# Shinokawa/Fast-SCNN-pytorch

Hardware: AMD Instinct MI355X
Metric: images/sec fwd+bwd @1024x2048 bs=8 per GPU; 1/2/4/8-GPU scaling (higher is better)
Workload: dtype bf16; 1 GPU; cfg3 train step: fwd + CE(ignore -1) + bwd + fused SGD (fused low-res upsample+CE head); model=FastSCNN (19 classes), global_batch=8, per_gpu_batch=8, parallelism=dp1

## Files before the change

### fast-scnn-pytorch_amd/_lib.py

```python
import ctypes
import os
import threading

_HERE = os.path.dirname(os.path.abspath(__file__))
LIB_PATH = os.environ.get("FSCNN_LIB", os.path.join(_HERE, "libfastscnn_hip.so"))

DT_F32, DT_BF16, DT_F16 = 0, 1, 2
DT_U8 = 3

c_int, c_ll, c_float, c_vp, c_char_p = (ctypes.c_int, ctypes.c_longlong, ctypes.c_float,
                                        ctypes.c_void_p, ctypes.c_char_p)
c_ull, c_double = ctypes.c_ulonglong, ctypes.c_double
P_int, P_ll, P_vp = ctypes.POINTER(c_int), ctypes.POINTER(c_ll), ctypes.POINTER(c_vp)
P_float = ctypes.POINTER(c_float)
P_double = ctypes.POINTER(c_double)
c_uint, P_ubyte = ctypes.c_uint, ctypes.POINTER(ctypes.c_ubyte)


class AuxHead(ctypes.Structure):
    _fields_ = [("head", c_int), ("aux_weight", c_float), ("ignore_index", c_ll),
                ("smooth", c_float), ("dice_weight", c_float), ("focal_weight", c_float),
                ("alpha", c_float), ("gamma", c_float), ("thresh", c_float), ("min_kept", c_ll),
                ("class_weight", c_vp)]

# ... 69 lines not shown
                               c_vp]),
    "fscnn_e2e_bev": (c_int, [c_vp, c_int, c_int, c_int, c_int, c_int, c_int, c_int, c_int, c_int,
                              c_int, P_double, c_int, c_int, c_int, c_vp, c_vp, c_vp]),
    "fscnn_forward_e2e_bev": (c_int, [c_vp, c_vp, c_int, c_int, c_int, c_int, c_int, P_float,
                                      P_float, c_int, c_int, c_int, P_double, c_int, c_int, c_int,
                                      c_vp, c_vp, c_vp, c_vp, c_vp, c_vp, c_vp]),
    "fscnn_path_plan": (c_int, [c_vp, c_int, c_int, P_path_params, c_vp, c_vp, c_vp]),
    "fscnn_overlay_mask": (c_int, [c_vp, c_int, c_int, c_int, c_int, c_int, c_vp, c_int, c_int,
                                   P_ubyte, c_vp, c_int, c_float, c_float, c_float, c_vp, c_vp,
                                   c_vp]),
    "fscnn_e2e_overlay": (c_int, [c_vp, c_int, c_int, c_int, c_int, c_int, c_int, c_int, c_int,
                                  c_int, c_int, c_vp, c_int, c_int, c_int, c_int, P_ubyte, c_uint,
                                  c_float, c_float, c_float, c_vp, c_vp, c_vp]),
    "fscnn_forward_e2e_overlay": (c_int, [c_vp, c_vp, c_int, c_int, c_int, c_int, c_int, P_float,
                                          P_float, c_int, c_int, c_int, P_ubyte, c_uint, c_float,
                                          c_float, c_float, c_vp, c_vp, c_vp, c_vp, c_vp, c_vp,
                                          c_vp]),
    "fscnn_seg_metric": (c_int, [c_vp, c_int, c_vp, c_ll, c_int, c_vp, c_vp]),
    "fscnn_forward_aux": (c_int, [c_vp, c_vp, c_int, c_vp, c_vp, c_int, c_vp, c_vp, c_vp, c_vp,
                                  c_ull, c_float, c_float, c_vp]),
    "fscnn_backward_aux": (c_int, [c_vp, c_vp, c_vp, c_vp, c_int, c_vp, c_vp, c_vp, c_vp, c_ull,
                                   c_float, c_int, c_int, c_vp]),
    "fscnn_forward_loss": (c_int, [c_vp, c_vp, c_int, c_vp, c_ll, c_vp, c_vp, c_vp, c_vp, c_vp,
                                   c_ull, c_float, c_float, c_vp]),
    "fscnn_backward_loss": (c_int, [c_vp, c_vp, c_vp, c_vp, c_int, c_vp, c_vp, c_vp, c_vp, c_ull,
                                    c_float, c_int, c_int, c_vp]),
    "fscnn_dice_head_ws_bytes": (c_ll, [c_vp]),
    "fscnn_forward_loss_dice": (c_int, [c_vp, c_vp, c_int, c_vp, c_float, c_float, c_float,
                                        c_float, c_float, c_vp, c_vp, c_vp, c_vp, c_vp, c_vp, c_vp,
                                        c_ull, c_float, c_float, c_vp]),
    "fscnn_backward_loss_dice": (c_int, [c_vp, c_vp, c_vp, c_float, c_float, c_float, c_vp, c_int,
                                         c_vp, c_vp, c_vp, c_vp, c_vp, c_ull, c_float, c_int,
                                         c_int, c_vp]),
    "fscnn_forward_loss_ohem": (c_int, [c_vp, c_vp, c_int, c_vp, c_ll, c_float, c_ll, c_vp, c_vp,
                                        c_vp, c_vp, c_vp, c_vp, c_vp, c_vp, c_vp, c_vp, c_ull,
                                        c_float, c_float, c_vp]),
    "fscnn_aux_head_ws_bytes": (c_ll, [c_vp, c_int]),
    "fscnn_aux_head_ws_offset": (c_ll, [c_vp, c_int, c_char_p, c_int]),
    "fscnn_forward_loss_aux": (c_int, [c_vp, c_vp, c_int, c_vp, P_aux_head, c_vp, c_vp, c_vp, c_vp,
                                       c_vp, c_vp, c_ull, c_float, c_float, c_vp]),
    "fscnn_backward_loss_aux": (c_int, [c_vp, c_vp, P_aux_head, c_vp, c_int, c_vp, c_int, c_vp,
                                        c_vp, c_vp, c_vp, c_vp, c_ull, c_float, c_int, c_int,
                                        c_vp]),
    "fscnn_backward_dx": (c_int, [c_vp, c_vp, c_vp, c_vp, c_vp, c_vp, c_int, c_vp, c_int, c_vp,
                                  c_vp, c_vp, c_vp, c_ull, c_float, c_int, c_int, c_vp]),
    "fscnn_prof_begin": (c_int, [c_int, c_int]),
    "fscnn_prof_end": (c_int, [ctypes.POINTER(ctypes.c_double), P_ll, ctypes.POINTER(ctypes.c_double),
                               ctypes.POINTER(ctypes.c_double)]),
    "fscnn_prof_launch": (c_int, [c_ll, ctypes.POINTER(c_int), ctypes.POINTER(ctypes.c_float),
                                  ctypes.POINTER(ctypes.c_double), ctypes.POINTER(ctypes.c_double),
                                  ctypes.POINTER(c_char_p)]),
    "fscnn_prof_kind_name": (c_char_p, [c_int]),
    "fscnn_ce_parts": (c_ll, [c_int, c_ll]),
    "fscnn_ce_fwd": (c_int, [c_vp, c_int, c_vp, c_int, c_int, c_ll, c_ll, c_vp, c_vp, c_vp]),
    "fscnn_ce_bwd": (c_int, [c_vp, c_int, c_vp, c_int, c_int, c_ll, c_ll, c_vp, c_vp, c_vp,
                             c_vp]),
    "fscnn_sgd": (c_int, [c_vp, c_vp, c_vp, c_ll, c_float, c_float, c_float, c_float, c_int,
                          c_int, c_float, c_vp]),
    "fscnn_adamw": (c_int, [c_vp, c_vp, c_vp, c_vp, c_vp, c_ll, c_double, c_double, c_double,
                            c_double, c_double, c_int, c_int, c_vp, c_int, c_vp, c_vp, c_vp]),
    "fscnn_adamw_segments": (c_int, [c_vp, c_vp, c_vp, c_vp, c_vp, c_vp, c_vp, c_int, c_vp, c_int,
                                     c_vp, c_int, c_vp, c_int, c_int, c_vp, c_vp, c_vp]),
    "fscnn_conv0_fwd": (c_int, [c_vp, c_int, c_int, c_int, c_int, c_vp, c_vp, c_vp, c_int, c_vp,
                                c_int, c_vp]),
    "fscnn_conv0_wgrad_slab_floats": (c_ll, [c_int, c_int, c_int]),
    "fscnn_conv0_wgrad": (c_int, [c_vp, c_int, c_int, c_int, c_int, c_vp, c_int, c_vp, c_vp, c_vp]),
    "fscnn_dw3x3_fwd": (c_int, [c_vp, c_int, c_int, c_int, c_int, c_int, c_int, c_vp, c_vp, c_vp,
                                c_int, c_vp, c_vp]),
    "fscnn_dw3x3_dgrad": (c_int, [c_vp, c_int, c_int, c_int, c_int, c_int, c_int, c_vp, c_vp,
                                  c_vp]),
    "fscnn_dw3x3_wgrad_slab_floats": (c_ll, [c_int, c_int, c_int, c_int, c_int, c_int]),
    "fscnn_dw3x3_wgrad": (c_int, [c_vp, c_vp, c_int, c_int, c_int, c_int, c_int, c_int, c_vp,
                                  c_vp, c_vp]),
    "fscnn_pw_gemm": (c_int, [c_int, c_int, c_int, c_vp, c_int, c_vp, c_int, c_int, c_vp, c_vp,
                              c_vp, c_int, c_int, c_vp, c_int, c_vp, c_int, c_vp]),
    "fscnn_pw_dgrad_bnbwd": (c_int, [c_int, c_int, c_int, c_vp, c_int, c_vp, c_int, c_vp, c_int,
                                     c_vp, c_int, c_vp, c_int, c_vp, c_vp, c_vp, c_vp, c_int,
                                     c_vp, c_vp, c_vp, c_vp, c_vp, c_vp, c_int, P_int, c_vp]),
    "fscnn_kth_smallest": (c_int, [c_vp, c_ll, c_ll, c_vp, c_vp, c_vp]),
    "fscnn_debug_stamps": (c_int, [c_vp, c_int]),
    "fscnn_debug_stamp_count": (c_int, []),
    "fscnn_debug_stamp_tag": (c_char_p, [c_int]),
    "fscnn_pw_wgrad_slab_floats": (c_ll, [c_int, c_int, c_int]),
    "fscnn_pw_gemm_stats_parts": (c_int, [c_int, c_int, c_int, c_int, c_int, c_int]),
    "fscnn_pw_wgrad": (c_int, [c_int, c_int, c_int, c_vp, c_int, c_vp, c_int, c_vp, c_vp, c_int,
                               c_vp]),
    "fscnn_bn_finalize": (c_int, [c_vp, c_int, c_int, c_vp, c_vp, c_vp, c_vp, c_vp, c_float,
                                  c_vp, c_vp, c_vp, c_vp, c_vp]),
    "fscnn_bilinear_ac_fwd": (c_int, [c_vp, c_int, c_int, c_int, c_int, c_int, c_int, c_int,
                                      c_vp, c_int, c_int, c_vp]),
    "fscnn_bilinear_ac_bwd": (c_int, [c_vp, c_int, c_int, c_int, c_int, c_int, c_int, c_int,
                                      c_vp, c_vp, c_vp]),
    "fscnn_pyramid_pool_fwd": (c_int, [c_vp, c_int, c_int, c_int, c_int, c_int, c_int, c_vp,
                                       c_vp]),
    "fscnn_block_ir_fwd": (c_int, [c_vp, c_int, c_int, c_int, c_int, c_int, c_int, c_int, c_int,
                                   c_vp, c_vp, c_vp, c_vp, c_vp, c_vp, c_vp, c_vp, c_vp, c_int,
                                   c_vp, c_int, c_vp]),
    "fscnn_pyramid_pool_bwd": (c_int, [c_vp, c_int, c_int, c_int, c_int, c_int, c_vp, c_int,
                                       c_int, c_vp]),
    "fscnn_bn_apply": (c_int, [c_ll, c_int, c_vp, c_int, c_vp, c_vp, c_vp, c_int, c_vp, c_vp, c_vp,
                               c_int, c_int, c_vp, c_int, c_int, c_vp]),
    "fscnn_bn_bwd": (c_int, [c_ll, c_int, c_vp, c_int, c_vp, c_int, c_vp, c_vp, c_vp, c_vp, c_vp,
                             c_int, c_int, c_vp, c_vp, c_vp, c_vp, c_vp, c_vp, c_vp, c_vp, c_vp,
                             c_vp, c_vp, c_vp, c_vp, c_int, P_int, P_int, c_vp]),
    "fscnn_ppm_branches_ok": (c_int, [c_int, c_int, c_int]),
    "fscnn_ppm_branches_fwd": (c_int, [c_int, P_int, c_int, c_vp, c_vp, c_vp, c_vp, c_vp, c_vp,
                                       c_vp, c_float, c_vp, c_vp, c_int, c_vp, c_vp, c_vp, c_vp,
                                       c_int, c_vp]),
    "fscnn_ppm_branches_bwd": (c_int, [c_int, P_int, c_int, c_vp, c_int, c_vp, c_int, c_vp, c_vp,
                                       c_vp, c_vp, c_vp, c_vp, c_vp, c_vp, c_vp, c_vp, c_vp, c_int,
                                       c_vp]),
    "fscnn_ppm_up_fwd": (c_int, [c_vp, c_int, c_int, c_int, c_int, c_vp, c_int, c_int, c_vp]),
    "fscnn_ppm_up_bwd": (c_int, [c_vp, c_int, c_int, c_int, c_int, c_int, c_int, c_vp, c_vp]),
    "fscnn_dropout": (c_int, [c_vp, c_int, c_int, c_int, c_int, c_int, c_int, c_ull, c_vp, c_ull,
                              c_float, c_vp, c_vp, c_vp, c_int, c_vp]),
    "fscnn_dw3x3_parts": (c_int, [c_int, c_int, c_int, c_int, c_int, c_int, c_int]),
    "fscnn_dw3x3_ct_width": (c_int, [c_int, c_int, c_int, c_int, c_int, c_int]),
    "fscnn_dw3x3_fwd_train": (c_int, [c_vp, c_int, c_int, c_int, c_int, c_int, c_int, c_vp, c_vp,
                                      c_vp, c_vp, c_vp, c_vp, c_vp, c_vp, c_vp, c_vp, c_vp, c_vp,
                                      c_float, c_vp, c_vp, c_vp, c_vp, P_int, c_vp]),
    "fscnn_dw3x3_dgrad_bn": (c_int, [c_vp, c_int, c_int, c_int, c_int, c_int, c_int, c_vp, c_vp,
                                     c_vp, c_vp, c_vp, c_vp, c_vp, c_int, c_vp, c_vp, c_vp, c_vp,
                                     c_vp, c_vp, P_int, c_vp]),
    "fscnn_dw3x3_wgrad_train": (c_int, [c_vp, c_vp, c_int, c_int, c_int, c_int, c_int, c_int,
                                        c_vp, c_vp, c_vp, c_vp, c_vp]),
    "fscnn_pw_fwd_train_route": (c_int, [c_int, c_int, c_int, c_int, c_int, c_int, c_int, P_int]),
    "fscnn_pw_fwd_train": (c_int, [c_int, c_int, c_int, c_vp, c_int, c_vp, c_vp, c_vp, c_int, c_vp,
                                   c_vp, c_int, c_vp, c_vp, c_vp, c_vp, c_vp, c_vp, c_vp, c_vp,
                                   c_float, c_vp, c_vp, c_vp, c_vp, c_int, P_int, P_int, c_vp]),
    "fscnn_pw_wgrad_train": (c_int, [c_int, c_int, c_int, c_vp, c_int, c_vp, c_int, c_vp, c_vp,
                                     c_vp, c_vp, c_vp, c_vp, c_int, P_int, c_vp]),
    "fscnn_pw_dgrad_train_route": (c_int, [c_int, c_int, c_int, c_int, c_int, c_int, c_int, c_int,
                                           P_int]),
    "fscnn_pw_dgrad_train": (c_int, [c_int, c_int, c_int, c_vp, c_int, c_vp, c_int, c_vp, c_int,
                                     c_vp, c_int, c_vp, c_int, c_vp, c_vp, c_vp, c_vp, c_int,
                                     c_vp, c_vp, c_vp, c_vp, c_vp, c_vp, c_vp, c_int, c_float,
                                     c_ull, c_ull, c_vp, c_int, P_int, P_int, c_vp]),
    "fscnn_im2col3": (c_int, [c_vp, c_int, c_int, c_int, c_int, c_int, c_int, c_vp, c_int, c_vp]),
    "fscnn_col2im3": (c_int, [c_vp, c_int, c_int, c_int, c_int, c_int, c_int, c_vp, c_int, c_int,
                              c_vp]),
    "fscnn_block_ir_s2_fwd": (c_int, [c_vp, c_int, c_int, c_int, c_int, c_int, c_int, c_int, c_int,
                                      c_vp, c_vp, c_vp, c_vp, c_vp, c_vp, c_vp, c_vp, c_vp, c_vp,
                                      c_int, c_vp]),
    "fscnn_block_ltd_fwd": (c_int, [c_vp, c_int, c_int, c_int, c_int, c_int, c_vp, c_vp, c_vp,
                                    c_vp, c_vp, c_vp, c_vp, c_vp, c_vp, c_vp, c_int, c_vp]),
    "fscnn_block_dsconv_fwd": (c_int, [c_vp, c_int, c_int, c_int, c_int, c_int, c_int, c_vp, c_vp,
                                       c_vp, c_vp, c_vp, c_vp, c_vp, c_int, c_vp]),
    "fscnn_block_dsconv_res_fwd": (c_int, [c_vp, c_int, c_int, c_int, c_int, c_int, c_int, c_int,
                                           c_int, c_vp, c_vp, c_vp, c_vp, c_vp, c_vp, c_vp, c_int,
                                           c_vp, c_int, c_vp]),
    "fscnn_block_cls_fwd": (c_int, [c_vp, c_int, c_int, c_int, c_int] + [c_vp] * 14 + [c_int, c_vp, c_vp,
                                                                              c_int, c_vp]),
    "fscnn_block_ffm_fwd": (c_int, [c_vp, c_int, c_int, c_int, c_int, c_int, c_int, c_vp, c_int,
                                    c_vp, c_vp, c_vp, c_vp, c_vp, c_vp, c_vp, c_vp, c_vp, c_vp,
                                    c_int, c_vp]),
}

_lib = None
_lock = threading.Lock()


def load():
    global _lib
    if _lib is not None:
        return _lib
    with _lock:
# ... 48 lines not shown
```

### fast-scnn-pytorch_amd/csrc/capi.cpp

```cpp
#include <algorithm>
#include <chrono>
#include <cmath>
#include <cstdlib>
#include <cstdarg>
#include <cstdio>
#include <cstring>
#include <new>
#include <string>

#include "../../include/fastscnn.h"
#include "net.hpp"

namespace fscnn {

static thread_local char g_err[512] = "";

void set_error(const char* fmt, ...) {
  va_list ap;
  va_start(ap, fmt);
  vsnprintf(g_err, sizeof g_err, fmt, ap);
  va_end(ap);
}
const char* last_error() { return g_err; }

// ... 1125 lines not shown
                      int dz_dtype, float* slab, float* dw, void* stream) {
  Conv0WgradArgs a{};
  a.x = x; a.x_bf16 = x_dtype; a.N = N; a.H = H; a.W = W;
  a.Ho = (H - 3) / 2 + 1; a.Wo = (W - 3) / 2 + 1; a.dz = dz; a.slab = slab;
  int rc = conv0_wgrad(a, dz_dtype, S(stream));
  if (rc) return rc;
  return reduce_slabs(slab, conv0_wgrad_parts(N, a.Ho, a.Wo, 0), 864, 864, dw, 0, S(stream));
}

int fscnn_dw3x3_fwd(const void* x, int dtype, int N, int H, int W, int C, int stride,
                    const float* w, const float* scale, const float* shift, int relu, void* y,
                    void* stream) {
  DwArgs a{};
  a.N = N; a.H = H; a.W = W; a.C = C; a.stride = stride;
  a.Ho = (H - 1) / stride + 1; a.Wo = (W - 1) / stride + 1;
  a.x = x; a.w = w; a.scale = scale; a.shift = shift; a.relu = relu; a.y = y;
  return dw_fwd(a, dtype, S(stream));
}
int fscnn_dw3x3_dgrad(const void* dy, int dtype, int N, int H, int W, int C, int stride,
                      const float* w, void* dx, void* stream) {
  DwBwdArgs a{};
  a.N = N; a.H = H; a.W = W; a.C = C; a.stride = stride;
  a.Ho = (H - 1) / stride + 1; a.Wo = (W - 1) / stride + 1;
  a.dy = dy; a.w = w; a.dx = dx;
  return dw_dgrad(a, dtype, S(stream));
}
long long fscnn_dw3x3_wgrad_slab_floats(int N, int H, int W, int C, int stride, int dtype) {
  int Ho = (H - 1) / stride + 1, Wo = (W - 1) / stride + 1;
  return (long long)dw_wgrad_parts(N, Ho, Wo, C, dtype, stride) * 9 * C;
}
int fscnn_dw3x3_wgrad(const void* x, const void* dy, int dtype, int N, int H, int W, int C,
                      int stride, float* slab, float* dw, void* stream) {
  DwBwdArgs a{};
  a.N = N; a.H = H; a.W = W; a.C = C; a.stride = stride;
  a.Ho = (H - 1) / stride + 1; a.Wo = (W - 1) / stride + 1;
  a.x = x; a.dy = dy; a.slab = slab;
  int rc = dw_wgrad(a, dtype, S(stream));
  if (rc) return rc;
  return dw_wgrad_reduce(slab, dw_wgrad_parts(N, a.Ho, a.Wo, C, dtype, stride), C, dw, S(stream));
}

int fscnn_pw_gemm_stats_parts(int M, int N, int K, int lda, int ldc, int dtype) {
  GemmArgs a{};
  static float dummy;
  a.M = M; a.N = N; a.K = K; a.lda = lda; a.ldb = K; a.ldc = ldc; a.part = &dummy;
  return gemm_nt_parts(a, dtype);
}
int fscnn_pw_gemm(int M, int N, int K, const void* A, int lda, const void* B, int ldb,
                  int b_trans, const float* scale, const float* shift, const void* R, int ldr,
                  int relu, void* C, int ldc, float* stats_part, int dtype, void* stream) {
  GemmArgs a{};
  a.M = M; a.N = N; a.K = K; a.A = A; a.lda = lda; a.B = B; a.ldb = ldb; a.b_trans = b_trans;
  a.scale = scale; a.shift = shift; a.R = R; a.ldr = ldr; a.relu = relu; a.C = C; a.ldc = ldc;
  a.part = stats_part;
  return gemm_nt(a, dtype, S(stream));
}
int fscnn_pw_dgrad_bnbwd(int M, int N, int K, const void* D, int ldd, const void* B, int ldb,
                         const void* R, int ldr, void* dX, int lddx, const void* z, int ldz,
                         const float* mean, const float* invstd, const float* scale,
                         const float* shift, int relu_mode, float* part, unsigned* counters,
                         double* tsum, float* dgamma, float* dbeta, float* coef, int dtype,
                         int* path, void* stream) {
  if (!D || !B || !dX || !z || !mean || !invstd || !scale || !shift || !part || !counters ||
      !tsum || !dgamma || !dbeta || !coef) {
    set_error("fscnn_pw_dgrad_bnbwd: null argument");
    return E_INVALID;
  }
  if (dtype < DT_F32 || dtype > DT_F16 || (relu_mode != 0 && relu_mode != 2)) {
    set_error("fscnn_pw_dgrad_bnbwd: dtype %d / relu_mode %d", dtype, relu_mode);
    return E_INVALID;
  }
  GemmArgs a{};
  a.M = M; a.N = N; a.K = K; a.A = D; a.lda = ldd; a.B = B; a.ldb = ldb; a.b_trans = 0;
  a.R = R; a.ldr = ldr; a.C = dX; a.ldc = lddx;
  a.bpart = part; a.bz = z; a.ldbz = ldz;
  a.bmean = mean; a.binvstd = invstd; a.bscale = scale; a.bshift = shift; a.bmode = relu_mode;
  a.tail.counters = counters; a.tail.tsum = tsum; a.tail.count = (double)M;
  a.tail.dgamma = dgamma; a.tail.dbeta = dbeta; a.tail.coef = coef;
  if (path) *path = gemm_stream_ok(a, dtype) ? 1 : 0;
  return gemm_nt(a, dtype, S(stream));
}
long long fscnn_pw_wgrad_slab_floats(int M, int N, int K) {
  return (long long)gemm_tn_splits(M, N, K) * N * K;
}
int fscnn_pw_wgrad(int M, int N, int K, const void* D, int ldd, const void* X, int ldx,
                   float* slab, float* dW, int dtype, void* stream) {
  GemmTnArgs a{};
  a.M = M; a.N = N; a.K = K; a.D = D; a.ldd = ldd; a.X = X; a.ldx = ldx; a.slab = slab;
  int s = gemm_tn_splits(M, N, K);
  int rc = gemm_tn(a, s, dtype, S(stream));
  if (rc) return rc;
  return reduce_slabs(slab, s, (long long)N * K, (long long)N * K, dW, 0, S(stream));
}

int fscnn_bn_finalize(float* part, int P, int C, const float* gamma, const float* beta,
                      float* rmean, float* rvar, long long* nbt, float momentum, float* mean,
                      float* invstd, float* scale, float* shift, void* stream) {
  BnFinalizeArgs a{};
  a.part = part; a.P = P; a.C = C; a.gamma = gamma; a.beta = beta; a.rmean = rmean;
  a.rvar = rvar; a.nbt = nbt; a.momentum = momentum; a.mean = mean; a.invstd = invstd;
  a.scale = scale; a.shift = shift;
  return bn_finalize(a, S(stream));
}

int fscnn_bilinear_ac_fwd(const void* x, int dtype, int N, int Hi, int Wi, int C, int Ho, int Wo,
                          void* y, int out_nchw, int out_dtype, void* stream) {
  UpArgs a{};
  a.N = N; a.Hi = Hi; a.Wi = Wi; a.C = C; a.Ho = Ho; a.Wo = Wo; a.x = x; a.ldx = C; a.y = y;
  a.ldy = C;
  if (out_nchw) return up_nchw(a, dtype, out_dtype, S(stream));
  return up_nhwc(a, dtype, S(stream));
}
int fscnn_bilinear_ac_bwd(const void* dy, int dtype, int N, int Hi, int Wi, int C, int Ho, int Wo,
                          float* tmp, void* dx, void* stream) {
  AxisBwdArgs a{};
  a.n_o1 = (long long)N * Ho; a.n_o2 = 1; a.Lout = Wo; a.Lin = Wi; a.n_in = C;
  a.g = dy; a.g_s1 = (long long)Wo * C; a.g_idx = C; a.g_in = 1;
  a.d = tmp; a.d_s1 = (long long)Wi * C; a.d_idx = C; a.d_in = 1;
  int rc = axis_bwd(a, dtype, DT_F32, S(stream));
  if (rc) return rc;
  AxisBwdArgs b{};
  b.n_o1 = N; b.n_o2 = 1; b.Lout = Ho; b.Lin = Hi; b.n_in = (long long)Wi * C;
  b.g = tmp; b.g_s1 = (long long)Ho * Wi * C; b.g_idx = (long long)Wi * C; b.g_in = 1;
  b.d = dx; b.d_s1 = (long long)Hi * Wi * C; b.d_idx = (long long)Wi * C; b.d_in = 1;
  return axis_bwd(b, DT_F32, dtype, S(stream));
}
int fscnn_pyramid_pool_fwd(const void* x, int dtype, int N, int H, int W, int C, int ldx,
                           void* pooled, void* stream) {
  PoolArgs a{};
  a.N = N; a.H = H; a.W = W; a.C = C; a.x = x; a.ldx = ldx; a.pooled = pooled;
  return pyramid_pool(a, dtype, S(stream));
}
int fscnn_pyramid_pool_bwd(const void* dpooled, int dtype, int N, int H, int W, int C, void* dx,
                           int lddx, int accumulate, void* stream) {
  PoolBwdArgs a{};
  a.N = N; a.H = H; a.W = W; a.C = C; a.dpooled = dpooled; a.dx = dx; a.lddx = lddx;
  a.accumulate = accumulate;
  return pyramid_pool_bwd(a, dtype, S(stream));
}

static bool dt_ok(int dtype) { return dtype >= DT_F32 && dtype <= DT_F16; }
static int vec_w(int dtype) { return dtype == DT_F32 ? 4 : 8; }
static bool ld_ok(int ld, int C, int V) { return ld >= C && ld % V == 0; }

int fscnn_bn_apply(long long M, int C, const void* z, int ldz, const float* scale,
                   const float* shift, const void* z2, int ldz2, const float* scale2,
                   const float* shift2, const void* res, int ldres, int relu, void* y, int ldy,
                   int dtype, void* stream) {
  if (!z || !scale || !shift || !y || (z2 && (!scale2 || !shift2))) {
    set_error("fscnn_bn_apply: null argument");
    return E_INVALID;
  }
  if (!dt_ok(dtype)) {
    set_error("fscnn_bn_apply: dtype %d", dtype);
    return E_INVALID;
  }
  const int V = vec_w(dtype);
  if (M < 1 || C < 1 || C % V || !ld_ok(ldz, C, V) || !ld_ok(ldy, C, V) ||
      (z2 && !ld_ok(ldz2, C, V)) || (res && !ld_ok(ldres, C, V)) ||
      M * (C / V) >= (1LL << 31)) {
    set_error("fscnn_bn_apply: M=%lld C=%d ldz=%d ldz2=%d ldres=%d ldy=%d (C and every row stride "
              "a multiple of %d, strides >= C)", M, C, ldz, ldz2, ldres, ldy, V);
    return E_INVALID;
  }
  BnApplyArgs a{};
  a.M = M; a.C = C;
// ... 826 lines not shown
```

### fast-scnn-pytorch_amd/csrc/gemm.hip

```cpp
#include "bn_finish.hpp"

namespace fscnn {


constexpr int G_BM = 128;
constexpr int G_VROW = 8;
constexpr int G_VPAD = 9;
constexpr int G_ATMAX = 768;

template <typename T>
struct MfmaOp;

template <>
struct MfmaOp<float> {
  static __device__ __forceinline__ void run(const uint4& a, const uint4& b, f32x4& acc) {
    acc = __builtin_amdgcn_mfma_f32_16x16x4f32(__uint_as_float(a.x), __uint_as_float(b.x), acc, 0, 0, 0);
    acc = __builtin_amdgcn_mfma_f32_16x16x4f32(__uint_as_float(a.y), __uint_as_float(b.y), acc, 0, 0, 0);
    acc = __builtin_amdgcn_mfma_f32_16x16x4f32(__uint_as_float(a.z), __uint_as_float(b.z), acc, 0, 0, 0);
    acc = __builtin_amdgcn_mfma_f32_16x16x4f32(__uint_as_float(a.w), __uint_as_float(b.w), acc, 0, 0, 0);
  }
};

template <>
struct MfmaOp<bf16> {
// ... 662 lines not shown
        rx[i][h] = *reinterpret_cast<const uint4*>(X + (okx ? (size_t)m * a.ldx + k : 0));
      }
    }
  };
  float xsc[XT ? V : 1], xsh[XT ? V : 1];
  if constexpr (XT) {
    const int kb = k0 + (tid % VPR) * V;
#pragma unroll
    for (int j = 0; j < V; ++j) {
      const int k = kb + j < a.K ? kb + j : 0;
      xsc[j] = a.x_scale[k];
      xsh[j] = a.x_shift[k];
    }
  }
  auto mask = [&](int mc) {
#pragma unroll
    for (int i = 0; i < PAIRS; ++i) {
      const int id = tid + 256 * i;
      const int rp = id / VPR, vv = id - rp * VPR;
      const int n = n0 + vv * V, k = k0 + vv * V;
#pragma unroll
      for (int h = 0; h < 2; ++h) {
        const bool okm = mc + 2 * rp + h < me;
        uint4 dv = rd[i][h];
        rd[i][h] = zero_tail<T>(dv, okm ? a.N - n : 0);
        uint4 xv = rx[i][h];
        if constexpr (XT) xv = bnrelu_vec<T>(xv, xsc, xsh);
        rx[i][h] = zero_tail<T>(xv, okm ? a.K - k : 0);
      }
    }
  };
  using Pair = typename std::conditional<sizeof(T) == 2, uint32_t, uint2>::type;
  if (mb < me) load(mb);
  for (int mc = mb; mc < me; mc += TN_MC) {
    mask(mc);
    __syncthreads();
#pragma unroll
    for (int i = 0; i < PAIRS; ++i) {
      const int id = tid + 256 * i;
      const int rp = id / VPR, vv = id - rp * VPR;
      const T* d0 = reinterpret_cast<const T*>(&rd[i][0]);
      const T* d1 = reinterpret_cast<const T*>(&rd[i][1]);
      const T* x0 = reinterpret_cast<const T*>(&rx[i][0]);
      const T* x1 = reinterpret_cast<const T*>(&rx[i][1]);
#pragma unroll
      for (int j = 0; j < V; ++j) {
        const int n = vv * V + j;
        const int off = n * LD + swz(n, 2 * rp);
        Pair pd, px;
        __builtin_memcpy(reinterpret_cast<T*>(&pd), d0 + j, sizeof(T));
        __builtin_memcpy(reinterpret_cast<T*>(&pd) + 1, d1 + j, sizeof(T));
        __builtin_memcpy(reinterpret_cast<T*>(&px), x0 + j, sizeof(T));
        __builtin_memcpy(reinterpret_cast<T*>(&px) + 1, x1 + j, sizeof(T));
        *reinterpret_cast<Pair*>(&sDt[off]) = pd;
        *reinterpret_cast<Pair*>(&sXt[off]) = px;
      }
    }
    __syncthreads();
    if (mc + TN_MC < me) load(mc + TN_MC);
#pragma unroll
    for (int ks = 0; ks < TN_MC / 32; ++ks) {
      const int kb = ks * 32 + 8 * lq;
#pragma unroll
      for (int i = 0; i < 2; ++i)
#pragma unroll
        for (int j = 0; j < 2; ++j) {
          const int na = wn + i * 16 + li, nb = wk + j * 16 + li;
          TnOps<T>::mma(&sDt[na * LD + swz(na, kb)], &sXt[nb * LD + swz(nb, kb)], acc[i][j]);
        }
    }
  }
  float* sl = a.slab + (size_t)split * a.N * a.K;
#pragma unroll
  for (int i = 0; i < 2; ++i)
#pragma unroll
    for (int j = 0; j < 2; ++j)
#pragma unroll
      for (int r = 0; r < 4; ++r) {
        int n = n0 + wn + i * 16 + lq * 4 + r, k = k0 + wk + j * 16 + li;
        if (n < a.N && k < a.K) sl[(size_t)n * a.K + k] = acc[i][j][r];
      }
}

int gemm_tn_splits(int M, int N, int K) {
  constexpr int target = 512;
  int tiles = cdiv(N, TN_T) * cdiv(K, TN_T);
  int s = target / tiles;
  int smax = cdiv(M, 4 * TN_MC);
  if (s > smax) s = smax;
  if (s >= 8) s &= ~7;
  if (s < 1) s = 1;
  return s;
}

int gemm_tn(GemmTnArgs a, int splits, int dtype, hipStream_t st) {
  const int V = dtype == DT_F32 ? 4 : 8;
  if (a.ldd % V || a.ldx % V || (uintptr_t)a.D % 16 || (uintptr_t)a.X % 16) {
    set_error("gemm_tn: operands must be 16-B aligned (ldd=%d ldx=%d)", a.ldd, a.ldx);
    return E_INVALID;
  }
  a.rows_per_split = cdiv(cdiv(a.M, splits), TN_MC) * TN_MC;
  a.splits = splits;
  dim3 grid(cdiv(a.N, TN_T) * cdiv(a.K, TN_T) * splits);
  const double E = dtype == DT_F32 ? 4.0 : 2.0;
  const double M = a.M, N = a.N, K = a.K;
  ProfScope ps(PK_GEMM_TN, st, E * (M * N + M * K) + 4.0 * N * K, 2.0 * M * N * K);
  const bool xt = a.x_scale != nullptr;
  if (xt && (!a.x_shift || a.K % V)) {
    set_error("gemm_tn: lazy BN on X needs x_shift and K %% %d == 0", V);
    return E_UNSUPPORTED;
  }
#define TN_LAUNCH(T)                                        \
  do {                                                      \
    if (xt) prof_launch(gemm_tn_kernel<T, true>, grid, 256, 0, st, a); \
    else prof_launch(gemm_tn_kernel<T, false>, grid, 256, 0, st, a);   \
  } while (0)
  if (dtype == DT_F32) TN_LAUNCH(float);
  else if (dtype == DT_F16) TN_LAUNCH(f16);
  else TN_LAUNCH(bf16);
#undef TN_LAUNCH
  return check_launch("gemm_tn");
}

constexpr int RED_Q = 64;

__global__ void reduce_fold_kernel(float* slab, int S, int Q, long long stride, int count) {
  int i = blockIdx.x * blockDim.x + threadIdx.x;
  int q = blockIdx.y;
  if (i >= count) return;
  float s = 0.f;
  for (int k0 = q; k0 < S; k0 += 8 * Q) {
    float v[8];
#pragma unroll
    for (int u = 0; u < 8; ++u) {
      const int k = k0 + u * Q;
      const float t = slab[(size_t)(k < S ? k : q) * stride + i];
      v[u] = k < S ? t : 0.f;
    }
#pragma unroll
    for (int u = 0; u < 8; ++u) s += v[u];
  }
  slab[(size_t)q * stride + i] = s;
}

__global__ void reduce_final_kernel(const float* slab, int S, long long stride, int count,
                                    float* out, int accumulate, int C9) {
  int i = blockIdx.x * blockDim.x + threadIdx.x;
  if (i >= count) return;
  float s = 0.f;
  for (int k0 = 0; k0 < S; k0 += 8) {
    float v[8];
#pragma unroll
    for (int u = 0; u < 8; ++u) {
      const float t = slab[(size_t)(k0 + u < S ? k0 + u : 0) * stride + i];
      v[u] = k0 + u < S ? t : 0.f;
    }
#pragma unroll
    for (int u = 0; u < 8; ++u) s += v[u];
  }
  int o = C9 ? (i % C9) * 9 + i / C9 : i;
  out[o] = accumulate ? out[o] + s : s;
}

int reduce_slabs_ex(float* slab, int S, long long stride, long long count, float* out,
                    int accumulate, int C9, hipStream_t st) {
  if (count <= 0 || count > 0x7fffffff) { set_error("reduce_slabs: bad count"); return E_INVALID; }
  int n = (int)count;
  int S2 = S;
  if (S > RED_Q) {
    dim3 g1(cdiv(n, 256), RED_Q);
    prof_launch(reduce_fold_kernel, g1, 256, 0, st, slab, S, RED_Q, stride, n);
    S2 = RED_Q;
  }
  prof_launch(reduce_final_kernel, cdiv(n, 256), 256, 0, st, slab, S2, stride, n, out, accumulate, C9);
  return check_launch("reduce_slabs");
}

int reduce_slabs(float* slab, int S, long long stride, long long count, float* out,
                 int accumulate, hipStream_t st) {
  return reduce_slabs_ex(slab, S, stride, count, out, accumulate, 0, st);
}

__device__ __forceinline__ int red_job(const RedTable& t, int b) {
  int lo = 0, hi = t.n - 1;
  while (lo < hi) {
    const int mid = (lo + hi + 1) >> 1;
    if (t.blk0[mid] <= b) lo = mid;
    else hi = mid - 1;
  }
  return lo;
}

__global__ void reduce_fold_multi_kernel(RedTable t) {
  const int jb = red_job(t, blockIdx.x);
  const RedJob& J = t.j[jb];
  const int nb = cdiv(J.count, 256);
  const int local = blockIdx.x - t.blk0[jb];
  const int q = local / nb;
  const int i = (local - q * nb) * blockDim.x + threadIdx.x;
  if (i >= J.count) return;
  float s = 0.f;
  for (int k0 = q; k0 < J.S; k0 += 8 * J.Q) {
// ... 95 lines not shown
```

### fast-scnn-pytorch_amd/csrc/kernels.hpp

```cpp
#pragma once
#include "common.hpp"

struct fscnn_path_params;

namespace fscnn {

constexpr int MAX_FOLD = 48;
constexpr double BN_FROZEN_COUNT = -1.0;


struct Conv0Args {
  const void* x;
  int x_bf16;
  int N, H, W, Ho, Wo;
  const float* w;
  const float* scale;
  const float* shift;
  int relu;
  void* y;
  float* part;
  unsigned long long* stamps = nullptr;
};

struct Conv0WgradArgs {
// ... 436 lines not shown
  const float *scp, *shp;
  void* y; int ldy;
  const void* r = nullptr;
  int ldr = 0;
  int rs;
  const void* wc = nullptr;
  const float* bc = nullptr;
  int ncls = 0;
  void* logits = nullptr; int ldl = 0;
  int Hi = 0, Wi = 0;
  const void* xh = nullptr;
  int ldxh = 0;
  const void* wh = nullptr;
  const float *sch = nullptr, *shh = nullptr;
  unsigned long long* stamps = nullptr;
};
bool ds_ok(const DsArgs& a);
struct Ds2Args {
  const void* x;
  int N, H, W, Ho, Wo;
  const float* wd;
  const float *scd, *shd;
  const void* wp;
  const float *scp, *shp;
  void* y; int ldy;
  unsigned long long* stamps = nullptr;
};
bool ds2_ok(const Ds2Args& a);
int ds2_fwd(const Ds2Args& a, int dtype, hipStream_t st);
int ds_rows(int N, int H, int W);
int ds_fwd(const DsArgs& a, int dtype, hipStream_t st);

struct Conv0DgradArgs {
  const void* dz;
  const float* w;
  int N, H, W, Ho, Wo;
  void* dx;
  int dx_dtype;
};
int conv0_dgrad(const Conv0DgradArgs& a, int dz_dtype, hipStream_t st);
int conv0_parts(int N, int Ho, int Wo);
int conv0_fwd(const Conv0Args& a, int y_dtype, hipStream_t st);
int conv0_wgrad_parts(int N, int Ho, int Wo, int rows_per_block);
int conv0_wgrad(const Conv0WgradArgs& a, int dz_dtype, hipStream_t st);

constexpr int LC0_SLAB = 2 * 864 + 27;
struct LtdC0BwdArgs {
  int N, H, W;
  int Ho, Wo;
  const void* dy;
  const float* w;
  BnBwdPart bs{};
  BnTail tail{};
  const void* x;
  int x_dtype, XH, XW;
  float* slab;
};
int ltd_c0_bwd_parts(int N, int H, int W);
bool ltd_c0_bwd_ok(int dtype, int x_dtype, int XW, const void* x);
int ltd_c0_bwd(const LtdC0BwdArgs& a, int dtype, hipStream_t st);
int conv0_wgrad_combine(const float* sums, const float* tab, const float* mean, float* dw,
                        hipStream_t st);

int dw_parts(int N, int Ho, int Wo, int C, int dtype, int stride);
int dw_ct_width(int N, int Ho, int Wo, int W, int C, int dtype, int stride);
int dw_fwd(const DwArgs& a, int dtype, hipStream_t st);
int dw_dgrad(const DwBwdArgs& a, int dtype, hipStream_t st);
int dw_dgrad_parts(int N, int H, int W, int C, int dtype, int stride);
int dw_fwd_tail_ink(const DwArgs& a, int dtype, int* P);
int dw_dgrad_tail_ink(const DwBwdArgs& a, int dtype, int* P);
int dw_wgrad_parts(int N, int Ho, int Wo, int C, int dtype, int stride);
int dw_wgrad(const DwBwdArgs& a, int dtype, hipStream_t st);
int dw_wgrad_reduce(float* slab, int P, int C, float* dw, hipStream_t st);

int gemm_parts(int M);
int gemm_nt(const GemmArgs& a, int dtype, hipStream_t st);
bool gemm_stream_ok(const GemmArgs& a, int dtype);
int gemm_stream(const GemmArgs& a, int dtype, hipStream_t st);
int gemm_stream_parts(const GemmArgs& a, int dtype);
int gemm_nt_parts(const GemmArgs& a, int dtype);
int gemm_nt_tail_ink(const GemmArgs& a, int dtype, int* P);
int gemm_tn_splits(int M, int N, int K);
int gemm_tn(GemmTnArgs a, int splits, int dtype, hipStream_t st);
int reduce_slabs(float* slab, int S, long long stride, long long count, float* out,
                 int accumulate, hipStream_t st);
int reduce_slabs_ex(float* slab, int S, long long stride, long long count, float* out,
                    int accumulate, int C9, hipStream_t st);
constexpr int RED_MAXJOBS = 64;
struct RedJob {
  float* slab;
  float* out;
  long long stride;
  int S, count, accumulate, C9;
  int Q = 0;
};
struct RedTable {
  int n = 0;
  int blocks = 0;
  int blk0[RED_MAXJOBS + 1] = {};
  RedJob j[RED_MAXJOBS];
};
int reduce_slabs_multi(const RedTable& t, hipStream_t st);
int colsum_parts(int M);
int colsum(const void* D, int M, int N, int ld, float* part, int dtype, hipStream_t st);

int bn_fold(const FoldTable& t, hipStream_t st);
int bn_finalize(const BnFinalizeArgs& a, hipStream_t st);
int bn_apply(const BnApplyArgs& a, int dtype, hipStream_t st);
int bn_bwd_parts(long long M, int C, int dtype, int* rows_per_block);
int bn_bwd_reduce(const BnBwdArgs& a, int dtype, hipStream_t st);
int bn_bwd_finalize(float* part, int P, int C, double count, float* dgamma, float* dbeta,
                    float* coef, hipStream_t st, unsigned* counters = nullptr,
                    const BnBwdTab& tab = BnBwdTab());
int bn_bwd_apply(const BnBwdArgs& a, int dtype, hipStream_t st);

int up_nhwc(const UpArgs& a, int dtype, hipStream_t st);
int up_nchw(const UpArgs& a, int in_dtype, int out_dtype, hipStream_t st);
bool up_nchw_rows_path(const UpArgs& a);
int up_argmax(const UpArgs& a, int in_dtype, void* labels, int label_u8, hipStream_t st);
int seg_metric(const void* pred, int pred_u8, const long long* target, long long n, int C,
               long long* counts, hipStream_t st);
int axis_bwd(const AxisBwdArgs& a, int g_dtype, int d_dtype, hipStream_t st);
int pyramid_pool(const PoolArgs& a, int dtype, hipStream_t st);
int pyramid_pool_bwd(const PoolBwdArgs& a, int dtype, hipStream_t st);
int ppm_up_fwd(const PpmUpArgs& a, int dtype, hipStream_t st);
int ppm_up_bwd(const PpmUpArgs& a, void* dfeats, int dtype, hipStream_t st);

bool ppm_branches_ok(int maxM, int K, int dtype);
int ppm_branches_fwd(const PpmFwdArgs& a, int dtype, hipStream_t st);
int ppm_branches_bwd(const PpmBwdArgs& a, int dtype, hipStream_t st);

int ce_parts(int N, long long HW);
int ce_fwd(const CeArgs& a, float* out, int dtype, hipStream_t st);
int ce_bwd(const CeArgs& a, const float* gout, const float* stats, int dtype, hipStream_t st);
int ohem_prob(const CeArgs& a, float thresh, float* prob, unsigned long long* counts, int dtype,
              hipStream_t st);
int ohem_threshold_dev(const float* key, long long n, const unsigned long long* counts,
                       long long min_kept, float thresh, unsigned* work, float* thr,
                       hipStream_t st);
int dice_loss_fwd(const void* logits, int dtype, const long long* target, int N, int C, long long HW,
                  float alpha, float gamma, int focal, float* part, double* stats, hipStream_t st);
int dice_loss_bwd(const void* logits, int dtype, const long long* target, int N, int C, long long HW,
                  float alpha, float gamma, int focal, const double* stats, const float* gout,
                  float smooth, float wd, float wf, void* dlogits, hipStream_t st);
int ce_head_parts(int N, int Hl, int Wl);
int ce_head(const CeHeadArgs& a, float* out2, int dtype, hipStream_t st);
bool ce_head2_form(int C, int ldl, int dtype);
bool ce_head_reads_tgt8(int C, int ldl, int W, int dtype);
int ce_pack_targets(const long long* t, long long n, int C, long long ignore_index,
                    signed char* out, hipStream_t st);
int ce_head_scale(const float* g_raw, void* g, long long M, int C, int ld, const float* gout,
                  const float* out2, int dtype, hipStream_t st, float weight = 1.f);
int aux_loss_combine(const float* main, const float* aux, float aux_weight, float* out3,
                     hipStream_t st);
long long dice_head_ws_bytes(int N, int Hl, int Wl, int C, int ldl);
int dice_head(const DiceHeadArgs& a, void* head_ws, float* loss, double* stats, int dtype,
              hipStream_t st);
int dice_head_scale(const void* head_ws, void* g, long long M, int C, int ld, const float* gout,
                    const double* stats, float smooth, float wd, float wf, double npix, int dtype,
                    hipStream_t st, float weight = 1.f);
bool ohem_head_ok(int C);
int ohem_head(const OhemHeadArgs& a, long long min_kept, unsigned* work, float* out2, int dtype,
              hipStream_t st);
int eval_head_parts(int N, int H, int W);
bool eval_head_ok(int N, int C, int Hl, int Wl, int H, int W, int dice);
int eval_head(const EvalHeadArgs& a, int dtype, hipStream_t st);
// ... 92 lines not shown
```

### include/fastscnn.h

```cpp
#ifndef FASTSCNN_H
#define FASTSCNN_H

#ifdef __cplusplus
extern "C" {
#endif

typedef struct fscnn_net fscnn_net;
typedef struct fscnn_plan fscnn_plan;

const char* fscnn_version(void);
const char* fscnn_last_error(void);

int fscnn_net_create(int num_classes, int aux, fscnn_net** out);
void fscnn_net_destroy(fscnn_net* net);
int fscnn_net_param_count(const fscnn_net* net, int* count, long long* total_floats);
int fscnn_net_param_info(const fscnn_net* net, int i, const char** name, long long* offset,
                         long long* numel);
int fscnn_net_buffer_count(const fscnn_net* net, int* count, long long* total_floats, int* num_bn);
int fscnn_net_buffer_info(const fscnn_net* net, int i, const char** name, long long* offset,
                          long long* numel);
int fscnn_net_stage_range(const fscnn_net* net, int stage, long long* begin, long long* end);

int fscnn_plan_create(const fscnn_net* net, int N, int H, int W, int dtype, int train,
                      fscnn_plan** out);
// ... 237 lines not shown
                               const void* res, int ldres, void* y, int ldy, void* stream);

int fscnn_block_cls_fwd(const void* x, int dtype, int N, int H, int W, const float* w_dw1,
                        const float* scale_d1, const float* shift_d1, const void* w_pw1,
                        const float* scale_p1, const float* shift_p1, const float* w_dw2,
                        const float* scale_d2, const float* shift_d2, const void* w_pw2,
                        const float* scale_p2, const float* shift_p2, const void* w_cls,
                        const float* b_cls, int ncls, void* tmp, void* logits, int ldl,
                        void* stream);

int fscnn_block_ffm_fwd(const void* low, int dtype, int N, int Hi, int Wi, int H, int W,
                        const void* high, int ldhigh, const float* w_dw, const float* scale_d,
                        const float* shift_d, const void* w_low, const float* scale_l,
                        const float* shift_l, const void* w_high, const float* scale_h,
                        const float* shift_h, void* y, int ldy, void* stream);

int fscnn_prof_begin(int kind, int max_launches);
int fscnn_prof_end(double* total_ms, long long* launches, double* bytes, double* flops);
int fscnn_prof_launch(long long i, int* kind, float* ms, double* bytes, double* flops,
                      const char** layer);
const char* fscnn_prof_kind_name(int kind);
int fscnn_debug_stamps(void* buf, int max_launches);
int fscnn_debug_stamp_count(void);
const char* fscnn_debug_stamp_tag(int i);

long long fscnn_ce_parts(int N, long long HW);
int fscnn_ce_fwd(const void* logits, int dtype, const long long* target, int N, int C,
                 long long HW, long long ignore_index, float* part, float* out2, void* stream);
int fscnn_ce_bwd(const void* logits, int dtype, const long long* target, int N, int C,
                 long long HW, long long ignore_index, const float* grad_out,
                 const float* out2, void* dlogits, void* stream);
int fscnn_sgd(float* p, const float* g, float* buf, long long n, float lr, float momentum,
              float dampening, float weight_decay, int nesterov, int first, float grad_scale,
              void* stream);

int fscnn_adamw(float* p, const float* g, float* exp_avg, float* exp_avg_sq,
                float* max_exp_avg_sq, long long n, double lr, double beta1, double beta2,
                double eps, double weight_decay, int amsgrad, int maximize, float* step, int tick,
                const float* grad_scale, const float* found_inf, void* stream);
#define FSCNN_ADAMW_CHUNK 2048
#define FSCNN_ADAMW_MAX_GROUPS 8
typedef struct fscnn_adamw_seg {
  long long begin, end;
  int group;
  int chunk0;
} fscnn_adamw_seg;
typedef struct fscnn_adamw_group {
  double lr, beta1, beta2, eps, weight_decay;
  int amsgrad, maximize;
  int step_slot;
} fscnn_adamw_group;
int fscnn_adamw_segments(float* p, const float* g, float* exp_avg, float* exp_avg_sq,
                         float* max_exp_avg_sq, const fscnn_adamw_seg* segs,
                         const fscnn_adamw_seg* host_segs, int nseg, const int* chunk_seg,
                         int nchunks, const fscnn_adamw_group* groups, int ngroups, float* steps,
                         int nslots, int tick, const float* grad_scale, const float* found_inf,
                         void* stream);

int fscnn_conv0_fwd(const void* x, int x_dtype, int N, int H, int W, const float* w,
                    const float* scale, const float* shift, int relu, void* y, int y_dtype,
                    void* stream);
long long fscnn_conv0_wgrad_slab_floats(int N, int H, int W);
int fscnn_conv0_wgrad(const void* x, int x_dtype, int N, int H, int W, const void* dz,
                      int dz_dtype, float* slab, float* dw, void* stream);
int fscnn_dw3x3_fwd(const void* x, int dtype, int N, int H, int W, int C, int stride,
                    const float* w, const float* scale, const float* shift, int relu, void* y,
                    void* stream);
int fscnn_dw3x3_dgrad(const void* dy, int dtype, int N, int H, int W, int C, int stride,
                      const float* w, void* dx, void* stream);
long long fscnn_dw3x3_wgrad_slab_floats(int N, int H, int W, int C, int stride, int dtype);
int fscnn_dw3x3_wgrad(const void* x, const void* dy, int dtype, int N, int H, int W, int C,
                      int stride, float* slab, float* dw, void* stream);
int fscnn_pw_gemm_stats_parts(int M, int N, int K, int lda, int ldc, int dtype);
int fscnn_pw_gemm(int M, int N, int K, const void* A, int lda, const void* B, int ldb,
                  int b_trans, const float* scale, const float* shift, const void* R, int ldr,
                  int relu, void* C, int ldc, float* stats_part, int dtype, void* stream);
int fscnn_pw_dgrad_bnbwd(int M, int N, int K, const void* D, int ldd, const void* B, int ldb,
                         const void* R, int ldr, void* dX, int lddx, const void* z, int ldz,
                         const float* mean, const float* invstd, const float* scale,
                         const float* shift, int relu_mode, float* part, unsigned* counters,
                         double* tsum, float* dgamma, float* dbeta, float* coef, int dtype,
                         int* path, void* stream);
long long fscnn_pw_wgrad_slab_floats(int M, int N, int K);
int fscnn_pw_wgrad(int M, int N, int K, const void* D, int ldd, const void* X, int ldx,
                   float* slab, float* dW, int dtype, void* stream);
int fscnn_bn_finalize(float* part, int P, int C, const float* gamma, const float* beta,
                      float* rmean, float* rvar, long long* nbt, float momentum, float* mean,
                      float* invstd, float* scale, float* shift, void* stream);
int fscnn_bilinear_ac_fwd(const void* x, int dtype, int N, int Hi, int Wi, int C, int Ho, int Wo,
                          void* y, int out_nchw, int out_dtype, void* stream);
int fscnn_bilinear_ac_bwd(const void* dy, int dtype, int N, int Hi, int Wi, int C, int Ho, int Wo,
                          float* tmp, void* dx, void* stream);
int fscnn_pyramid_pool_fwd(const void* x, int dtype, int N, int H, int W, int C, int ldx,
                           void* pooled, void* stream);
int fscnn_pyramid_pool_bwd(const void* dpooled, int dtype, int N, int H, int W, int C, void* dx,
                           int lddx, int accumulate, void* stream);

int fscnn_bn_apply(long long M, int C, const void* z, int ldz, const float* scale,
                   const float* shift, const void* z2, int ldz2, const float* scale2,
                   const float* shift2, const void* res, int ldres, int relu, void* y, int ldy,
                   int dtype, void* stream);
int fscnn_bn_bwd(long long M, int C, const void* dy, int lddy, const void* mask, int ldmask,
                 const void* z, const float* mean, const float* invstd, const float* scale,
                 const float* shift, int relu_mode, int frozen, const void* z2,
                 const float* mean2, const float* invstd2, const float* scale2, float* part,
                 unsigned* counters, void* dz, void* dz2, float* dgamma, float* dbeta,
                 float* dgamma2, float* dbeta2, float* coef, int dtype, int* P,
                 int* rows_per_block, void* stream);
int fscnn_ppm_branches_ok(int maxM, int K, int dtype);
int fscnn_ppm_branches_fwd(int nb, const int* M, int K, const void* x, const void* w,
                           const float* gamma, const float* beta, float* rmean, float* rvar,
                           long long* nbt, float momentum, void* z, void* y, int ldy, float* mean,
                           float* invstd, float* scale, float* shift, int dtype, void* stream);
int fscnn_ppm_branches_bwd(int nb, const int* M, int K, const void* dy, int lddy, const void* y,
                           int ldy, const void* z, const float* mean, const float* invstd,
                           const float* scale, const float* gamma, const void* x, const void* w,
                           float* dgamma, float* dbeta, float* dw, void* dx, int dtype,
                           void* stream);
int fscnn_ppm_up_fwd(const void* feats, int dtype, int N, int H, int W, void* y, int ldy, int coff,
                     void* stream);
int fscnn_ppm_up_bwd(const void* dy, int dtype, int N, int H, int W, int ldy, int coff,
                     void* dfeats, void* stream);
int fscnn_dropout(const void* x, int ldx, int dtype, int N, int H, int W, int C,
                  unsigned long long seed, const unsigned long long* seed_slot,
                  unsigned long long seed_add, float p, const float* x_scale,
                  const float* x_shift, void* y, int ldy, void* stream);
int fscnn_dw3x3_parts(int N, int H, int W, int C, int stride, int dtype, int dgrad);
int fscnn_dw3x3_ct_width(int N, int H, int W, int C, int stride, int dtype);
int fscnn_dw3x3_fwd_train(const void* x, int dtype, int N, int H, int W, int C, int stride,
                          const float* w, const float* in_scale, const float* in_shift, void* z,
                          float* part, unsigned* counters, double* tsum, const float* gamma,
                          const float* beta, float* rmean, float* rvar, long long* nbt,
                          float momentum, float* mean, float* invstd, float* scale, float* shift,
                          int* in_kernel, void* stream);
int fscnn_dw3x3_dgrad_bn(const void* dy, int dtype, int N, int H, int W, int C, int stride,
                         const float* w, void* dx, const void* z, const float* mean,
                         const float* invstd, const float* scale, const float* shift,
                         int relu_mode, float* part, unsigned* counters, double* tsum,
                         float* dgamma, float* dbeta, float* coef, int* in_kernel, void* stream);
int fscnn_dw3x3_wgrad_train(const void* x, const void* dy, int dtype, int N, int H, int W, int C,
                            int stride, const float* x_scale, const float* x_shift, float* slab,
                            float* dw, void* stream);

int fscnn_pw_fwd_train_route(int M, int N, int K, int lda, int ldc, int lazy, int dtype,
                             int* records);
int fscnn_pw_fwd_train(int M, int N, int K, const void* A, int lda, const float* a_scale,
                       const float* a_shift, const void* B, int ldb, const float* bias, void* z,
                       int ldc, float* part, unsigned* counters, double* tsum, const float* gamma,
                       const float* beta, float* rmean, float* rvar, long long* nbt,
                       float momentum, float* mean, float* invstd, float* scale, float* shift,
                       int dtype, int* route, int* records, void* stream);
int fscnn_pw_wgrad_train(int M, int N, int K, const void* D, int ldd, const void* X, int ldx,
                         const float* x_scale, const float* x_shift, float* slab, float* dW,
                         float* bias_part, float* dbias, int dtype, int* splits, void* stream);
int fscnn_pw_dgrad_train_route(int M, int N, int K, int ldd, int lddx, int residual, int drop_hw,
                               int dtype, int* records);
int fscnn_pw_dgrad_train(int M, int N, int K, const void* D, int ldd, const void* B, int ldb,
                         const void* R, int ldr, void* dX, int lddx, const void* z, int ldz,
                         const float* mean, const float* invstd, const float* scale,
                         const float* shift, int relu_mode, float* part, unsigned* counters,
                         double* tsum, float* dgamma, float* dbeta, float* coef, float* tab,
                         int drop_hw, float drop_p, unsigned long long seed,
                         unsigned long long seed_add, const unsigned long long* seed_slot,
                         int dtype, int* route, int* records, void* stream);
int fscnn_im2col3(const void* x, int ldx, int dtype, int N, int H, int W, int C, void* col,
                  int ldcol, void* stream);
// ... 8 lines not shown
```

Baseline: 1513 images/s.

## Add transpose-read LDS path with 16x16x32 MFMA for pointwise weight-gradient GEMM

Adds a new TN weight-gradient kernel for 16-bit dtypes. It stages D and X tiles into swizzled LDS images, reads them back with ds_read_tr16 transpose loads, and feeds the wider 16x16x32 bf16/f16 MFMA. Global loads are software-pipelined through a register ring with a double-buffered LDS. The aim is to cut LDS transpose and shuffle overhead and the MFMA instruction count in the wgrad reduction. It becomes the default for bf16/f16, with an env var to fall back to the old kernel. This adds complexity, and the swizzle and tail handling need to be correct.

```diff
diff --git a/fast-scnn-pytorch_amd/_lib.py b/fast-scnn-pytorch_amd/_lib.py
--- a/fast-scnn-pytorch_amd/_lib.py
+++ b/fast-scnn-pytorch_amd/_lib.py
@@ -175,6 +175,7 @@
     "fscnn_debug_stamp_count": (c_int, []),
     "fscnn_debug_stamp_tag": (c_char_p, [c_int]),
     "fscnn_pw_wgrad_slab_floats": (c_ll, [c_int, c_int, c_int]),
+    "fscnn_pw_wgrad_form": (c_int, [c_int, c_int, c_int, c_int]),
     "fscnn_pw_gemm_stats_parts": (c_int, [c_int, c_int, c_int, c_int, c_int, c_int]),
     "fscnn_pw_wgrad": (c_int, [c_int, c_int, c_int, c_vp, c_int, c_vp, c_int, c_vp, c_vp, c_int,
                                c_vp]),
diff --git a/fast-scnn-pytorch_amd/csrc/capi.cpp b/fast-scnn-pytorch_amd/csrc/capi.cpp
--- a/fast-scnn-pytorch_amd/csrc/capi.cpp
+++ b/fast-scnn-pytorch_amd/csrc/capi.cpp
@@ -1231,6 +1231,13 @@
 }
 long long fscnn_pw_wgrad_slab_floats(int M, int N, int K) {
   return (long long)gemm_tn_splits(M, N, K) * N * K;
+}
+int fscnn_pw_wgrad_form(int M, int N, int K, int dtype) {
+  if (M < 1 || N < 1 || K < 1 || dtype < DT_F32 || dtype > DT_F16) {
+    set_error("fscnn_pw_wgrad_form: M=%d N=%d K=%d dtype %d", M, N, K, dtype);
+    return -1;
+  }
+  return gemm_tn_form(dtype);
 }
 int fscnn_pw_wgrad(int M, int N, int K, const void* D, int ldd, const void* X, int ldx,
                    float* slab, float* dW, int dtype, void* stream) {
diff --git a/fast-scnn-pytorch_amd/csrc/gemm.hip b/fast-scnn-pytorch_amd/csrc/gemm.hip
--- a/fast-scnn-pytorch_amd/csrc/gemm.hip
+++ b/fast-scnn-pytorch_amd/csrc/gemm.hip
@@ -768,6 +768,153 @@
       }
 }
 
+constexpr int TN_RING = 2;
+constexpr int TN_IMG = TN_MC * TN_T * 2;
+
+__device__ __forceinline__ int tn_tr_swz(int r) { return (r & 2) | ((r & 8) >> 1); }
+
+__device__ __forceinline__ i16x8 tn_tr_read(const unsigned char* img, int off) {
+  typedef __attribute__((address_space(3))) i16x4 lds_i16x4;
+  const i16x4 lo = __builtin_amdgcn_ds_read_tr16_b64_v4i16((lds_i16x4*)(img + off));
+  const i16x4 hi = __builtin_amdgcn_ds_read_tr16_b64_v4i16((lds_i16x4*)(img + off + 4 * 2 * TN_T));
+  return __builtin_shufflevector(lo, hi, 0, 1, 2, 3, 4, 5, 6, 7);
+}
+
+template <typename T>
+__device__ __forceinline__ void tn_tr_mma(const i16x8& a, const i16x8& b, f32x4& acc) {
+  if constexpr (std::is_same<T, f16>::value) {
+    h16x8 ah, bh;
+    __builtin_memcpy(&ah, &a, 16);
+    __builtin_memcpy(&bh, &b, 16);
+    acc = __builtin_amdgcn_mfma_f32_16x16x32_f16(ah, bh, acc, 0, 0, 0);
+  } else {
+    acc = __builtin_amdgcn_mfma_f32_16x16x32_bf16(a, b, acc, 0, 0, 0);
+  }
+}
+
+template <typename T, bool XT, int R>
+__global__ __launch_bounds__(256, 4) void gemm_tn_tr_kernel(GemmTnArgs a) {
+  static_assert(sizeof(T) == 2 && TN_T == 64 && TN_MC == 64, "16-bit operands, 64 x 64 images");
+  constexpr int V = 8;
+  __shared__ __attribute__((aligned(16))) unsigned char s_img[2][2][TN_IMG];
+  const int tid = threadIdx.x, lane = tid & 63, wave = tid >> 6;
+  const int li = lane & 15, lq = lane >> 4;
+  const int tiles_k = cdiv(a.K, TN_T);
+  int split, tile;
+  xcd_tile(blockIdx.x, a.splits, cdiv(a.N, TN_T) * tiles_k, split, tile);
+  const int tn = tile / tiles_k, tk = tile - tn * tiles_k;
+  const int n0 = tn * TN_T, k0 = tk * TN_T;
+  const int wn = (wave >> 1) * 32, wk = (wave & 1) * 32;
+  const int mb = split * a.rows_per_split;
+  const int me = min(a.M, mb + a.rows_per_split);
+  const T* D = (const T*)a.D;
+  const T* X = (const T*)a.X;
+
+  f32x4 acc[2][2];
+#pragma unroll
+  for (int i = 0; i < 2; ++i)
+#pragma unroll
+    for (int j = 0; j < 2; ++j) acc[i][j] = f32x4{0.f, 0.f, 0.f, 0.f};
+
+  const int sv = tid & 7, sr = tid >> 3;
+  const int n = n0 + sv * V, k = k0 + sv * V;
+  const int st_off = sr * (2 * TN_T) + ((sv ^ tn_tr_swz(sr)) << 4);
+  auto load = [&](uint4 (&d)[2], uint4 (&x)[2], int mc) {
+#pragma unroll
+    for (int h = 0; h < 2; ++h) {
+      const int m = mc + sr + 32 * h;
+      const bool okd = m < me && n < a.N, okx = m < me && k < a.K;
+      d[h] = *reinterpret_cast<const uint4*>(D + (okd ? (size_t)m * a.ldd + n : 0));
+      x[h] = *reinterpret_cast<const uint4*>(X + (okx ? (size_t)m * a.ldx + k : 0));
+    }
+  };
+  float xsc[XT ? V : 1], xsh[XT ? V : 1];
+  if constexpr (XT) {
+#pragma unroll
+    for (int j = 0; j < V; ++j) {
+      const int kk = k + j < a.K ? k + j : 0;
+      xsc[j] = a.x_scale[kk];
+      xsh[j] = a.x_shift[kk];
+    }
+  }
+  const uint4 ones = make_uint4(~0u, ~0u, ~0u, ~0u);
+  const uint4 dm = zero_tail<T>(ones, a.N - n), xm = zero_tail<T>(ones, a.K - k);
+  auto keep = [](const uint4& v, const uint4& m, uint32_t r) {
+    return make_uint4(v.x & m.x & r, v.y & m.y & r, v.z & m.z & r, v.w & m.w & r);
+  };
+  auto stage = [&](int buf, const uint4 (&d)[2], const uint4 (&x)[2], int mc) {
+#pragma unroll
+    for (int h = 0; h < 2; ++h) {
+      const uint32_t rm = mc + sr + 32 * h < me ? ~0u : 0u;
+      uint4 xv = x[h];
+      if constexpr (XT) xv = bnrelu_vec<T>(xv, xsc, xsh);
+      const int off = st_off + 32 * h * (2 * TN_T);
+      *reinterpret_cast<uint4*>(&s_img[buf][0][off]) = keep(d[h], dm, rm);
+      *reinterpret_cast<uint4*>(&s_img[buf][1][off]) = keep(xv, xm, rm);
+    }
+  };
+  const int rr = 8 * lq + (li >> 2);
+  const int rd_row = rr * (2 * TN_T) + (li & 1) * 8, rd_swz = tn_tr_swz(rr), rd_ch = (li & 3) >> 1;
+  int offd[2], offx[2];
+#pragma unroll
+  for (int i = 0; i < 2; ++i) {
+    offd[i] = rd_row + (((((wn + 16 * i) >> 3) + rd_ch) ^ rd_swz) << 4);
+    offx[i] = rd_row + (((((wk + 16 * i) >> 3) + rd_ch) ^ rd_swz) << 4);
+  }
+  auto mma = [&](int buf) {
+#pragma unroll
+    for (int ks = 0; ks < TN_MC / 32; ++ks) {
+      i16x8 av[2], bv[2];
+#pragma unroll
+      for (int i = 0; i < 2; ++i) {
+        av[i] = tn_tr_read(s_img[buf][0], offd[i] + ks * 32 * (2 * TN_T));
+        bv[i] = tn_tr_read(s_img[buf][1], offx[i] + ks * 32 * (2 * TN_T));
+      }
+#pragma unroll
+      for (int i = 0; i < 2; ++i)
+#pragma unroll
+        for (int j = 0; j < 2; ++j) tn_tr_mma<T>(av[i], bv[j], acc[i][j]);
+    }
+  };
+
+  if (mb < me) {
+    const int nch = cdiv(me - mb, TN_MC);
+    uint4 rd[R][2], rx[R][2];
+#pragma unroll
+    for (int s = 0; s < R; ++s) load(rd[s], rx[s], mb + s * TN_MC);
+    stage(0, rd[0], rx[0], mb);
+    load(rd[0], rx[0], mb + R * TN_MC);
+    for (int c = 0; c < nch; c += R) {
+#pragma unroll
+      for (int s = 0; s < R; ++s) {
+        const int ci = c + s;
+        const int sn = (s + 1) % R;
+        __syncthreads();
+        stage((ci + 1) & 1, rd[sn], rx[sn], mb + (ci + 1) * TN_MC);
+        load(rd[sn], rx[sn], mb + (ci + 1 + R) * TN_MC);
+        if (ci < nch) mma(ci & 1);
+      }
+    }
+  }
+  float* sl = a.slab + (size_t)split * a.N * a.K;
+#pragma unroll
+  for (int i = 0; i < 2; ++i)
+#pragma unroll
+    for (int j = 0; j < 2; ++j)
+#pragma unroll
+      for (int r = 0; r < 4; ++r) {
+        int nn = n0 + wn + i * 16 + lq * 4 + r, kk = k0 + wk + j * 16 + li;
+        if (nn < a.N && kk < a.K) sl[(size_t)nn * a.K + kk] = acc[i][j][r];
+      }
+}
+
+static bool tn_generic() {
+  static const bool on = env_on("FSCNN_TN_GENERIC", false);
+  return on;
+}
+
+int gemm_tn_form(int dtype) { return dtype != DT_F32 && !tn_generic() ? 1 : 0; }
+
 int gemm_tn_splits(int M, int N, int K) {
   constexpr int target = 512;
   int tiles = cdiv(N, TN_T) * cdiv(K, TN_T);
@@ -801,9 +948,18 @@
     if (xt) prof_launch(gemm_tn_kernel<T, true>, grid, 256, 0, st, a); \
     else prof_launch(gemm_tn_kernel<T, false>, grid, 256, 0, st, a);   \
   } while (0)
-  if (dtype == DT_F32) TN_LAUNCH(float);
+#define TN_TR_LAUNCH(T)                                                        \
+  do {                                                                         \
+    if (xt) prof_launch(gemm_tn_tr_kernel<T, true, TN_RING>, grid, 256, 0, st, a); \
+    else prof_launch(gemm_tn_tr_kernel<T, false, TN_RING>, grid, 256, 0, st, a);   \
+  } while (0)
+  if (gemm_tn_form(dtype)) {
+    if (dtype == DT_F16) TN_TR_LAUNCH(f16);
+    else TN_TR_LAUNCH(bf16);
+  } else if (dtype == DT_F32) TN_LAUNCH(float);
   else if (dtype == DT_F16) TN_LAUNCH(f16);
   else TN_LAUNCH(bf16);
+#undef TN_TR_LAUNCH
 #undef TN_LAUNCH
   return check_launch("gemm_tn");
 }
diff --git a/fast-scnn-pytorch_amd/csrc/kernels.hpp b/fast-scnn-pytorch_amd/csrc/kernels.hpp
--- a/fast-scnn-pytorch_amd/csrc/kernels.hpp
+++ b/fast-scnn-pytorch_amd/csrc/kernels.hpp
@@ -542,6 +542,7 @@
 int gemm_nt_tail_ink(const GemmArgs& a, int dtype, int* P);
 int gemm_tn_splits(int M, int N, int K);
 int gemm_tn(GemmTnArgs a, int splits, int dtype, hipStream_t st);
+int gemm_tn_form(int dtype);
 int reduce_slabs(float* slab, int S, long long stride, long long count, float* out,
                  int accumulate, hipStream_t st);
 int reduce_slabs_ex(float* slab, int S, long long stride, long long count, float* out,
diff --git a/include/fastscnn.h b/include/fastscnn.h
--- a/include/fastscnn.h
+++ b/include/fastscnn.h
@@ -343,6 +343,7 @@
                          double* tsum, float* dgamma, float* dbeta, float* coef, int dtype,
                          int* path, void* stream);
 long long fscnn_pw_wgrad_slab_floats(int M, int N, int K);
+int fscnn_pw_wgrad_form(int M, int N, int K, int dtype);
 int fscnn_pw_wgrad(int M, int N, int K, const void* D, int ldd, const void* X, int ldx,
                    float* slab, float* dW, int dtype, void* stream);
 int fscnn_bn_finalize(float* part, int P, int C, const float* gamma, const float* beta,
```

Result: no change. 1506 images/s (-0.5%).
